# l90lpa/fv3-jedi-linearmodel

Hardware: AMD Instinct MI355X
Metric: column-updates/s per TL+AD dyn step (higher is better)
Workload: dtype f64; 1 GPU; C192L127 hydrostatic TL+AD, six cube faces dealt over 1 GPU(s) (6 per rank), table-driven exchange (221184 columns per GPU), k_split=2 n_split=6 dt=450s nq=4, hord mt/vt/tm/dp/tr=2/2/2/2/2 (sponge: 1/1/1/1 below level 9), kord=17, nord=1; columns_per_gpu=221184

## Files before the change

### fv3_jedi_linearmodel_amd/csrc/tpad.h

```cpp
#pragma once
#include "tpfused.h"

namespace fv3 {
FV3LM_LINK void run_tp_ad(Exec& ex, const TpFusedArgs& a0, const Ctx& c);
}

#if !defined(FV3LM_SPLIT_BUILD) || defined(FV3LM_IMPL_TPAD)
namespace fv3 {

#ifndef FV3LM_TPD_H
#define FV3LM_TPD_H 32
#endif
#if defined(FV3LM_TPD_NOUNROLL) && !defined(FV3LM_HOST_EMUL)
#define TPD_LOOP(e, n) _Pragma("nounroll") for (int e = tid; e < (n); e += NTH)
#define TPD_LOOPU(e, u, n, E) _Pragma("nounroll") for (int e = tid, u = 0; e < (n); e += NTH)
#define TPD_QACC_DIRECT 1
#else
#define TPD_LOOP(e, n) TPF_LOOP(e, n)
#define TPD_LOOPU(e, u, n, E) TPF_LOOPU(e, u, n, E)
#define TPD_QACC_DIRECT 0
#endif
#ifndef FV3LM_TPD_PREFETCH
#define FV3LM_TPD_PREFETCH 1
#endif
#ifndef FV3LM_TPD_EXP
#define FV3LM_TPD_EXP 0
#endif
#ifndef FV3LM_TPD_THREADS
#define FV3LM_TPD_THREADS 1024
#endif
constexpr int TPD_W = 64, TPD_H = FV3LM_TPD_H;
constexpr int TPD_QW = TPD_W + 6, TPD_QH = TPD_H + 6;
constexpr int TPD_AW = TPD_W + 12, TPD_AH = TPD_H + 12;
constexpr int TPD_NQ = TPD_QW * TPD_QH;
constexpr int TPD_NF2 = TPD_QW * (TPD_QH + 1);
constexpr int TPD_NFA = (TPD_AW * TPD_QH > TPD_AH * TPD_QW ? TPD_AW * TPD_QH : TPD_AH * TPD_QW);
constexpr int TPD_NC = TPD_NFA;
constexpr int TPD_NT = 2 * TPD_NQ + TPD_NF2 + 2 * TPD_NFA + TPD_NC;
constexpr int TPD_THREADS = FV3LM_TPD_THREADS;

DEV double tps_al(double fm, double f0, double fp, double cm, double c0, double cp) {
  double s = (c0 > 0. ? (1. - c0) * (1. - c0) : (1. + c0) * (1. + c0)) * f0;
  if (cp > 0.) s -= cp * (1. - cp) * fp;
  if (!(cm > 0.)) s += cm * (1. + cm) * fm;
  return s;
}
template <class D>
DEV double tps_w(bool face, int x, int n1, const D& da, int k) {
  const int e = k - x + 2;
  if (e < 0 || e > 3) return 0.;
  if (!face || (x >= 3 && x <= n1 - 2)) return (e == 0 || e == 3) ? P2 : P1;
  double w[4]; ppm_w(face, x, n1, da, w);
  return w[e];
}
template <class D>
DEV double tps_q(int iord, bool face, int k, int n1, double f0, double fp, double c0, double cp, const double* al, const D& da) {
  double s = 0.;
  if (cp > 0.) s += (iord == 1 ? 1. : cp * (3. - 2. * cp)) * fp;
  if (!(c0 > 0.)) s += (iord == 1 ? 1. : -c0 * (3. + 2. * c0)) * f0;
  if (iord == 1) return s;
  if (!face || (k >= 4 && k <= n1 - 4)) return s + P2 * al[0] + P1 * al[1] + P1 * al[2] + P2 * al[3];
// ... 24 lines not shown
  const double dsc = -Z - (1. - sc) * Y;
  dc = up ? dsc : -dsc;
}

template <int NTH>
DEV void tp_ad_block(const TpFusedArgs& a, const Ctx& c, int tile, int k, int bx, int by, double* lds, int tid, int nth) {
  (void)nth;
  const Geom& g = c.g;
  const int nx = g.nx, ny = g.ny;
  const int is = g.is(), ie = g.ie(), js = g.js(), je = g.je();
  const bool face = g.face != 0;
  const int I0 = is + bx * TPD_W, I1 = (I0 + TPD_W - 1 < ie) ? I0 + TPD_W - 1 : ie;
  const int J0 = js + by * TPD_H, J1 = (J0 + TPD_H - 1 < je) ? J0 + TPD_H - 1 : je;
  const bool firstx = bx == 0, lastx = I1 == ie, firsty = by == 0, lasty = J1 == je;
  const int GI0 = firstx ? I0 - 3 : I0, GI1 = lastx ? I1 + 3 : I1, GJ0 = firsty ? J0 - 3 : J0, GJ1 = lasty ? J1 + 3 : J1;
  const size_t base = (size_t)(tile * a.nk + k - 1) * g.plane;
  auto at = [&](int i, int j) -> size_t { return base + g.idx(i, j); };
  const int iord = hord_of(c.lev[k - 1], a.hsel);
  double* Q = lds;
  double* QG = lds + TPD_NQ;
  double* F2 = lds + 2 * TPD_NQ;
  double* FA = F2 + TPD_NF2;
  double* AL = FA + TPD_NFA;
  double* CT = AL + TPD_NFA;
  auto cxe = [&](int i, int j) { return (j - (J0 - 3)) * TPD_AW + (i - (I0 - 6)); };
  auto cye = [&](int i, int j) { return (j - (J0 - 6)) * TPD_QW + (i - (I0 - 3)); };
  auto load_cx = [&](int e) -> double { const int i = I0 - 6 + e % TPD_AW, j = J0 - 3 + e / TPD_AW; return (i >= is && i <= ie + 1 && i <= I1 + 6 && j <= J1 + 3) ? a.crx.t[at(i, j)] : 0.; };
  auto load_cy = [&](int e) -> double { const int i = I0 - 3 + e % TPD_QW, j = J0 - 6 + e / TPD_QW; return (j >= js && j <= je + 1 && j <= J1 + 6 && i <= I1 + 3) ? a.cry.t[at(i, j)] : 0.; };
#if defined(FV3LM_HOST_EMUL) || defined(FV3LM_TPD_NOUNROLL)
  constexpr bool PRE = false;
#else
  constexpr bool PRE = FV3LM_TPD_PREFETCH != 0;
#endif
#define TPD_PF(arr, u, expr) (PRE ? arr[u] : (expr))
  constexpr int E_AQ = (TPD_AW * TPD_QH + NTH - 1) / NTH, E_QA = (TPD_QW * TPD_AH + NTH - 1) / NTH, E_Q = (TPD_NQ + NTH - 1) / NTH,
                E_V = (TPD_QW * (TPD_H + 1) + NTH - 1) / NTH, E_F = ((TPD_W + 1) * TPD_H + NTH - 1) / NTH,
                E_FB = (TPD_W * (TPD_H + 1) + NTH - 1) / NTH, E_I = (TPD_QW * TPD_H + NTH - 1) / NTH, E_J = (TPD_W * TPD_QH + NTH - 1) / NTH,
                E_G = (TPD_QW * (TPD_QH - 1) + NTH - 1) / NTH, E_GB = ((TPD_QW - 1) * TPD_QH + NTH - 1) / NTH;
#define TPD_SLOTS(E) (PRE ? (E) : 1)
  auto qe = [&](int i, int j) { return (j - (J0 - 3)) * TPD_QW + (i - (I0 - 3)); };
  auto corner_cell = [&](int i, int j) { return face && (i < 1 || i > nx) && (j < 1 || j > ny); };
  constexpr int EQ = (TPD_NQ + NTH - 1) / NTH;
  double qacc[EQ];

  auto cl = [](int m, int n1) { return m < 1 ? 1 : (m > n1 ? n1 : m); };
  (void)cl;
  { constexpr int n = TPD_NQ;
    TPD_LOOP(e, n) { const int i = I0 - 3 + e % TPD_QW, j = J0 - 3 + e / TPD_QW; Q[e] = (i <= I1 + 3 && j <= J1 + 3) ? a.q.t[at(i, j)] : 0.; } }

  {
    auto f2e = [&](int i, int j) { return (j - (J0 - 2)) * TPD_QW + (i - (I0 - 3)); };
    auto fae = [&](int i, int j) { return (j - (J0 - 3)) * TPD_AW + (i - (I0 - 6)); };
    auto ale = [&](int i, int j) { return (j - (J0 - 5)) * TPD_QW + (i - (I0 - 3)); };
    { constexpr int n = TPD_AW * TPD_QH;
      TPD_LOOP(e, n) {
        const int i = I0 - 6 + e % TPD_AW, j = J0 - 3 + e / TPD_AW;
        FA[e] = (i >= is && i <= ie + 1 && j >= js && j <= je && i <= I1 + 6 && j <= J1 + 3) ? 0.5 * a.mx.t[at(i, j)] * a.fx.p[at(i, j)] : 0.;
        CT[e] = load_cx(e);
      } }
    double cv[TPD_SLOTS(E_V)];
    if constexpr (PRE) { constexpr int n = TPD_QW * (TPD_H + 1);
      TPD_LOOPU(e, u, n, E_V) { const int i = I0 - 3 + e % TPD_QW, j = J0 + e / TPD_QW; cv[u] = (i <= I1 + 3 && j <= J1 + 1) ? a.cry.t[at(i, j)] : 0.; } }
    TPF_SYNC();
    double ar2[TPD_SLOTS(E_I)], y02[TPD_SLOTS(E_I)], y12[TPD_SLOTS(E_I)], ry2[TPD_SLOTS(E_I)];
    if constexpr (PRE) { constexpr int n = TPD_QW * TPD_H;
      TPD_LOOPU(e, u, n, E_I) { const int i = I0 - 3 + e % TPD_QW, j = J0 + e / TPD_QW; const bool in = i <= I1 + 3 && j <= J1;
        ar2[u] = in ? MET(area, i, j) : 0.; y02[u] = in ? a.yfx.t[at(i, j)] : 0.; y12[u] = in ? a.yfx.t[at(i, j + 1)] : 0.; ry2[u] = in ? a.ray.t[at(i, j)] : 1.; } }
    { constexpr int n = TPD_QW * (TPD_H + 1);
      TPD_LOOPU(e, u, n, E_V) {
        const int i = I0 - 3 + e % TPD_QW, j = J0 + e / TPD_QW;
        if (i > I1 + 3 || j > J1 + 1) continue;
        auto line = [&](int jj) -> double { int ii = i, j2 = jj; if (face) corner_map(g, 2, ii, j2); return Q[qe(ii, j2)]; };
        const MetY da{c.m.dya, c, tile, i};
        if (FV3LM_TPD_EXP && (a.exp & 1)) { F2[f2e(i, j)] = line(j) * TPD_PF(cv, u, a.cry.t[at(i, j)]); continue; }
        const double cc = TPD_PF(cv, u, a.cry.t[at(i, j)]);
        if (iord == 2 && !(face && (i < 1 || i > nx) && (j <= 3 || j >= ny - 1))) { double v_, d_; tpd_flux2<TPD_QW>(face, j, ny + 1, Q + qe(i, j), cc, da, v_, d_); F2[f2e(i, j)] = v_; }
        else F2[f2e(i, j)] = ppm_flux<double>(iord, face, j, ny + 1, line, da, cc);
      } }
    TPF_SYNC();
    double fx3[TPD_SLOTS(E_F)];
    if constexpr (PRE) { constexpr int w = TPD_W + 1, n = w * TPD_H;
      TPD_LOOPU(e, u, n, E_F) { const int i = I0 + e % w, j = J0 + e / w; fx3[u] = (j <= J1 && (i <= I1 || (lastx && i == I1 + 1))) ? a.fx.p[at(i, j)] : 0.; } }
    { constexpr int n = TPD_QW * TPD_H;
      TPD_LOOPU(e, u, n, E_I) {
        const int i = I0 - 3 + e % TPD_QW, j = J0 + e / TPD_QW;
        if (i > I1 + 3 || j > J1) continue;
        QG[qe(i, j)] = (Q[qe(i, j)] * TPD_PF(ar2, u, MET(area, i, j)) + TPD_PF(y02, u, a.yfx.t[at(i, j)]) * F2[f2e(i, j)] - TPD_PF(y12, u, a.yfx.t[at(i, j + 1)]) * F2[f2e(i, j + 1)]) / TPD_PF(ry2, u, a.ray.t[at(i, j)]);
      } }
    TPF_SYNC();
    double ry4[TPD_SLOTS(E_Q)], ar4[TPD_SLOTS(E_Q)], ro4[TPD_SLOTS(E_Q)];
    if constexpr (PRE) { constexpr int n = TPD_NQ;
      TPD_LOOPU(e, u, n, E_Q) { const int i = I0 - 3 + e % TPD_QW, j = J0 - 3 + e / TPD_QW;
        const bool in = i >= GI0 && i <= GI1 && j >= js && j <= je && j <= J1 + 3, own = in && j >= J0 && j <= J1;
        ry4[u] = in ? a.ray.t[at(i, j)] : 1.; ar4[u] = in ? MET(area, i, j) : 0.; ro4[u] = own ? a.ray.p[at(i, j)] : 0.; } }
    auto FX = [&](int m, int j) { return FA[fae(m, j)]; };
    { constexpr int w = TPD_W + 1, n = w * TPD_H;
      TPD_LOOPU(e, u, n, E_F) {
        const int i = I0 + e % w, j = J0 + e / w;
        if (j > J1 || !(i <= I1 || (lastx && i == I1 + 1))) continue;
        const double fo = FX(i, j), fxad = TPD_PF(fx3, u, a.fx.p[at(i, j)]);
        if (fo == 0. && fxad == 0.) continue;
        if (FV3LM_TPD_EXP && (a.exp & 2)) continue;
        auto line = [&](int ii) -> Dual { return Dual(QG[qe(ii, j)], 0.); };
        const MetX da{c.m.dxa, c, tile, j};
        Dual fl;
        if (iord == 2) tpd_flux2<1>(face, i, nx + 1, QG + qe(i, j), CT[cxe(i, j)], da, fl.v, fl.d);
        else fl = ppm_flux<Dual>(iord, face, i, nx + 1, line, da, Dual(CT[cxe(i, j)], 1.));
        a.crx.p[at(i, j)] += fl.d * fo;
        a.mx.p[at(i, j)] += 0.5 * fl.v * fxad;
      } }
    if (iord == 2 && !(FV3LM_TPD_EXP && (a.exp & 4))) {
      constexpr int n = TPD_AW * TPD_QH;
      TPD_LOOP(e, n) {
        const int x = I0 - 6 + e % TPD_AW, j = J0 - 3 + e / TPD_AW;
        double s = 0.;
        if (x >= I0 - 4 && x <= I1 + 5 && j >= js && j <= je && j <= J1 + 3) s = tps_al(FA[e - 1], FA[e], FA[e + 1], CT[e - 1], CT[e], CT[e + 1]);
        AL[e] = s;
      } }
    TPF_SYNC();
    double yf5[TPD_SLOTS(E_G)], fy5[TPD_SLOTS(E_G)], mm5[TPD_SLOTS(E_G)];
    if constexpr (PRE) { constexpr int n = TPD_QW * (TPD_QH - 1);
      TPD_LOOPU(e, u, n, E_G) { const int i = I0 - 3 + e % TPD_QW, m = J0 - 2 + e / TPD_QW;
        const bool on = i >= GI0 && i <= GI1 && m >= js && m <= je + 1 && m <= J1 + 3, in = on && i >= is && i <= ie;
        yf5[u] = on ? a.yfx.t[at(i, m)] : 0.; fy5[u] = in ? a.fy.p[at(i, m)] : 0.; mm5[u] = in ? a.my.t[at(i, m)] : 0.; } }
    { constexpr int n = TPD_NQ;
      TPD_LOOPU(e, u, n, EQ) {
        const int i = I0 - 3 + e % TPD_QW, j = J0 - 3 + e / TPD_QW;
        double s = 0., acc = 0.;
        if (i >= GI0 && i <= GI1 && j >= js && j <= je && j <= J1 + 3) {
          const bool own = j >= J0 && j <= J1;
          const double ry = TPD_PF(ry4, u, a.ray.t[at(i, j)]), ar = TPD_PF(ar4, u, MET(area, i, j)), rold = TPD_PF(ro4, u, own ? a.ray.p[at(i, j)] : 0.);
          const MetX da{c.m.dxa, c, tile, j};
          const int b0 = fae(i, j);
          if (iord == 333) {
            const double f[4] = {FA[b0 - 1], FA[b0], FA[b0 + 1], FA[b0 + 2]};
            const double cc[4] = {CT[b0 - 1], CT[b0], CT[b0 + 1], CT[b0 + 2]};
            s = tps_q333(face, i, nx + 1, f, cc, da);
          } else {
            const double al[4] = {AL[b0 - 1], AL[b0], AL[b0 + 1], AL[b0 + 2]};
            if (!(FV3LM_TPD_EXP && (a.exp & 8))) s = tps_q(iord, face, i, nx + 1, FA[b0], FA[b0 + 1], CT[b0], CT[b0 + 1], al, da);
          }
          s = s / ry;
          if (own) { a.ray.p[at(i, j)] = rold - QG[e] * s; acc = ar * s; }
        }
        if (TPD_QACC_DIRECT) { if (acc != 0.) a.q.p[at(i, j)] += acc; } else qacc[u] = acc;
        QG[e] = s;
      } }
    TPF_SYNC();
    double cyt[TPD_SLOTS(E_QA)], qo7[TPD_SLOTS(E_Q)];
    if constexpr (PRE) {
      { constexpr int n = TPD_QW * TPD_AH; TPD_LOOPU(e, u, n, E_QA) cyt[u] = load_cy(e); }
      { constexpr int n = TPD_NQ; TPD_LOOPU(e, u, n, E_Q) { const int i = I0 - 3 + e % TPD_QW, j = J0 - 3 + e / TPD_QW;
          qo7[u] = (i < GI0 || i > GI1 || j < GJ0 || j > GJ1 || corner_cell(i, j) || i > I1 + 3 || j > J1 + 3) ? 0. : a.q.p[at(i, j)]; } }
    }
    { constexpr int n = TPD_QW * (TPD_QH - 1);
      TPD_LOOPU(e, u, n, E_G) {
        const int i = I0 - 3 + e % TPD_QW, m = J0 - 2 + e / TPD_QW;
        double s = 0.;
        if (i >= GI0 && i <= GI1 && m >= js && m <= je + 1 && m <= J1 + 3) {
          const bool in = i >= is && i <= ie, own = m >= J0 && (m <= J1 || (lasty && m == J1 + 1));
          const double yf = TPD_PF(yf5, u, a.yfx.t[at(i, m)]), fyad = TPD_PF(fy5, u, in ? a.fy.p[at(i, m)] : 0.), mm = TPD_PF(mm5, u, in ? a.my.t[at(i, m)] : 0.);
          const double dg = (m <= je ? QG[qe(i, m)] : 0.) - (m >= js + 1 ? QG[qe(i, m - 1)] : 0.);
          s = yf * dg + 0.5 * mm * fyad;
          if (own) {
            const double f2v = F2[e];
            a.yfx.p[at(i, m)] += f2v * dg;
            if (in) a.my.p[at(i, m)] += 0.5 * f2v * fyad;
          }
        }
        F2[e] = s;
      } }
    { constexpr int n = TPD_QW * TPD_AH;
      TPD_LOOPU(e, u, n, E_QA) CT[e] = TPD_PF(cyt, u, load_cy(e)); }
    TPF_SYNC();
    auto FY2 = [&](int i, int m) { return (m >= J0 - 2 && m <= J1 + 3) ? F2[f2e(i, m)] : 0.; };
    if (iord == 2 && !(FV3LM_TPD_EXP && (a.exp & 4))) {
      constexpr int n = TPD_QW * TPD_AH;
      TPD_LOOP(e, n) {
        const int i = I0 - 3 + e % TPD_QW, x = J0 - 5 + e / TPD_QW;
        double s = 0.;
        if (i >= GI0 && i <= GI1 && x >= J0 - 4 && x <= J1 + 5) s = tps_al(FY2(i, x - 1), FY2(i, x), FY2(i, x + 1), CT[e], CT[e + TPD_QW], CT[e + 2 * TPD_QW]);
        AL[e] = s;
      } }
    TPF_SYNC();
    { constexpr int n = TPD_NQ;
      TPD_LOOPU(e, u, n, EQ) {
        const int i = I0 - 3 + e % TPD_QW, j = J0 - 3 + e / TPD_QW;
        const double acc = TPD_QACC_DIRECT ? 0. : qacc[u];
        if (i < GI0 || i > GI1 || j < GJ0 || j > GJ1 || corner_cell(i, j)) continue;
        const double qold = TPD_PF(qo7, u, a.q.p[at(i, j)]);
        const MetY da{c.m.dya, c, tile, i};
        const int cb = cye(i, j);
        double s;
        if (iord == 333) {
          const double f[4] = {FY2(i, j - 1), FY2(i, j), FY2(i, j + 1), FY2(i, j + 2)};
          const double cc[4] = {CT[cb - TPD_QW], CT[cb], CT[cb + TPD_QW], CT[cb + 2 * TPD_QW]};
          s = tps_q333(face, j, ny + 1, f, cc, da);
        } else {
          const int b0 = ale(i, j);
          const double al[4] = {AL[b0 - TPD_QW], AL[b0], AL[b0 + TPD_QW], AL[b0 + 2 * TPD_QW]};
          if (!(FV3LM_TPD_EXP && (a.exp & 8))) s = tps_q(iord, face, j, ny + 1, FY2(i, j), FY2(i, j + 1), CT[cb], CT[cb + TPD_QW], al, da);
        }
        a.q.p[at(i, j)] = qold + (acc + s);
      } }
    { constexpr int n = TPD_QW * (TPD_H + 1);
      TPD_LOOP(e, n) {
        const int i = I0 - 3 + e % TPD_QW, m = J0 + e / TPD_QW;
        if (i < GI0 || i > GI1 || !(m <= J1 || (lasty && m == J1 + 1))) continue;
        const double f = F2[f2e(i, m)];
        if (f == 0.) continue;
        if (FV3LM_TPD_EXP && (a.exp & 2)) continue;
        auto line = [&](int jj) -> Dual { int ii = i, j2 = jj; if (face) corner_map(g, 2, ii, j2); return Dual(Q[qe(ii, j2)], 0.); };
        const MetY da{c.m.dya, c, tile, i};
        double v_, d_;
        if (iord == 2 && !(face && (i < 1 || i > nx) && (m <= 3 || m >= ny - 1))) tpd_flux2<TPD_QW>(face, m, ny + 1, Q + qe(i, m), CT[cye(i, m)], da, v_, d_);
        else d_ = ppm_flux<Dual>(iord, face, m, ny + 1, line, da, Dual(CT[cye(i, m)], 1.)).d;
        a.cry.p[at(i, m)] += d_ * f;
      } }
    TPF_SYNC();
  }

  {
    auto f2e = [&](int i, int j) { return (j - (J0 - 3)) * (TPD_QW + 1) + (i - (I0 - 2)); };
    auto fae = [&](int i, int j) { return (j - (J0 - 6)) * TPD_QW + (i - (I0 - 3)); };
    auto ale = [&](int i, int j) { return (j - (J0 - 3)) * TPD_AW + (i - (I0 - 5)); };
    { constexpr int n = TPD_QW * TPD_AH;
      TPD_LOOP(e, n) {
        const int i = I0 - 3 + e % TPD_QW, j = J0 - 6 + e / TPD_QW;
        FA[e] = (j >= js && j <= je + 1 && i >= is && i <= ie && j <= J1 + 6 && i <= I1 + 3) ? 0.5 * a.my.t[at(i, j)] * a.fy.p[at(i, j)] : 0.;
      } }
    double ar2[TPD_SLOTS(E_J)], x02[TPD_SLOTS(E_J)], x12[TPD_SLOTS(E_J)], rx2[TPD_SLOTS(E_J)];
    if constexpr (PRE) { constexpr int n = TPD_W * TPD_QH;
      TPD_LOOPU(e, u, n, E_J) { const int i = I0 + e % TPD_W, j = J0 - 3 + e / TPD_W; const bool in = i <= I1 && j <= J1 + 3;
        ar2[u] = in ? MET(area, i, j) : 0.; x02[u] = in ? a.xfx.t[at(i, j)] : 0.; x12[u] = in ? a.xfx.t[at(i + 1, j)] : 0.; rx2[u] = in ? a.rax.t[at(i, j)] : 1.; } }
    { constexpr int w = TPD_W + 1, n = w * TPD_QH;
      TPD_LOOP(e, n) {
        const int i = I0 + e % w, j = J0 - 3 + e / w;
        if (i > I1 + 1 || j > J1 + 3) continue;
        auto line = [&](int ii) -> double { int i2 = ii, jj = j; if (face) corner_map(g, 1, i2, jj); return Q[qe(i2, jj)]; };
        const MetX da{c.m.dxa, c, tile, j};
        if (FV3LM_TPD_EXP && (a.exp & 1)) { F2[f2e(i, j)] = line(i) * a.crx.t[at(i, j)]; continue; }
        const double cc = a.crx.t[at(i, j)];
        if (iord == 2 && !(face && (j < 1 || j > ny) && (i <= 3 || i >= nx - 1))) { double v_, d_; tpd_flux2<1>(face, i, nx + 1, Q + qe(i, j), cc, da, v_, d_); F2[f2e(i, j)] = v_; }
        else F2[f2e(i, j)] = ppm_flux<double>(iord, face, i, nx + 1, line, da, cc);
      } }
    TPF_SYNC();
    double fy3[TPD_SLOTS(E_FB)];
    if constexpr (PRE) { constexpr int n = TPD_W * (TPD_H + 1);
      TPD_LOOPU(e, u, n, E_FB) { const int i = I0 + e % TPD_W, j = J0 + e / TPD_W; fy3[u] = (i <= I1 && (j <= J1 || (lasty && j == J1 + 1))) ? a.fy.p[at(i, j)] : 0.; } }
    { constexpr int n = TPD_W * TPD_QH;
      TPD_LOOPU(e, u, n, E_J) {
        const int i = I0 + e % TPD_W, j = J0 - 3 + e / TPD_W;
        if (i > I1 || j > J1 + 3) continue;
        QG[qe(i, j)] = (Q[qe(i, j)] * TPD_PF(ar2, u, MET(area, i, j)) + TPD_PF(x02, u, a.xfx.t[at(i, j)]) * F2[f2e(i, j)] - TPD_PF(x12, u, a.xfx.t[at(i + 1, j)]) * F2[f2e(i + 1, j)]) / TPD_PF(rx2, u, a.rax.t[at(i, j)]);
      } }
    TPF_SYNC();
    double rx4[TPD_SLOTS(E_Q)], ar4[TPD_SLOTS(E_Q)], ro4[TPD_SLOTS(E_Q)];
    if constexpr (PRE) { constexpr int n = TPD_NQ;
      TPD_LOOPU(e, u, n, E_Q) { const int i = I0 - 3 + e % TPD_QW, j = J0 - 3 + e / TPD_QW;
        const bool in = j >= GJ0 && j <= GJ1 && i >= is && i <= ie && i <= I1 + 3, own = in && i >= I0 && i <= I1;
        rx4[u] = in ? a.rax.t[at(i, j)] : 1.; ar4[u] = in ? MET(area, i, j) : 0.; ro4[u] = own ? a.rax.p[at(i, j)] : 0.; } }
    auto FY = [&](int i, int m) { return FA[fae(i, m)]; };
    { constexpr int n = TPD_W * (TPD_H + 1);
      TPD_LOOPU(e, u, n, E_FB) {
        const int i = I0 + e % TPD_W, j = J0 + e / TPD_W;
        if (i > I1 || !(j <= J1 || (lasty && j == J1 + 1))) continue;
        const double fo = FY(i, j), fyad = TPD_PF(fy3, u, a.fy.p[at(i, j)]);
        if (fo == 0. && fyad == 0.) continue;
        if (FV3LM_TPD_EXP && (a.exp & 2)) continue;
        auto line = [&](int jj) -> Dual { return Dual(QG[qe(i, jj)], 0.); };
        const MetY da{c.m.dya, c, tile, i};
        Dual fl;
        if (iord == 2) tpd_flux2<TPD_QW>(face, j, ny + 1, QG + qe(i, j), CT[cye(i, j)], da, fl.v, fl.d);
        else fl = ppm_flux<Dual>(iord, face, j, ny + 1, line, da, Dual(CT[cye(i, j)], 1.));
        a.cry.p[at(i, j)] += fl.d * fo;
        a.my.p[at(i, j)] += 0.5 * fl.v * fyad;
      } }
    if (iord == 2 && !(FV3LM_TPD_EXP && (a.exp & 4))) {
      constexpr int n = TPD_QW * TPD_AH;
      TPD_LOOP(e, n) {
        const int i = I0 - 3 + e % TPD_QW, x = J0 - 6 + e / TPD_QW;
        double s = 0.;
        if (x >= J0 - 4 && x <= J1 + 5 && i >= is && i <= ie && i <= I1 + 3) s = tps_al(FA[e - TPD_QW], FA[e], FA[e + TPD_QW], CT[e - TPD_QW], CT[e], CT[e + TPD_QW]);
        AL[e] = s;
      } }
    TPF_SYNC();
    double xf5[TPD_SLOTS(E_GB)], fx5[TPD_SLOTS(E_GB)], mm5[TPD_SLOTS(E_GB)];
    if constexpr (PRE) { constexpr int w = TPD_QW - 1, n = w * TPD_QH;
      TPD_LOOPU(e, u, n, E_GB) { const int m = I0 - 2 + e % w, j = J0 - 3 + e / w;
        const bool on = j >= GJ0 && j <= GJ1 && m >= is && m <= ie + 1 && m <= I1 + 3, in = on && j >= js && j <= je;
        xf5[u] = on ? a.xfx.t[at(m, j)] : 0.; fx5[u] = in ? a.fx.p[at(m, j)] : 0.; mm5[u] = in ? a.mx.t[at(m, j)] : 0.; } }
    { constexpr int n = TPD_NQ;
      TPD_LOOPU(e, u, n, EQ) {
        const int i = I0 - 3 + e % TPD_QW, j = J0 - 3 + e / TPD_QW;
        double s = 0., acc = 0.;
        if (j >= GJ0 && j <= GJ1 && i >= is && i <= ie && i <= I1 + 3) {
          const bool own = i >= I0 && i <= I1;
          const double rx = TPD_PF(rx4, u, a.rax.t[at(i, j)]), ar = TPD_PF(ar4, u, MET(area, i, j)), rold = TPD_PF(ro4, u, own ? a.rax.p[at(i, j)] : 0.);
          const MetY da{c.m.dya, c, tile, i};
          const int b0 = fae(i, j);
          if (iord == 333) {
            const double f[4] = {FA[b0 - TPD_QW], FA[b0], FA[b0 + TPD_QW], FA[b0 + 2 * TPD_QW]};
            const double cc[4] = {CT[b0 - TPD_QW], CT[b0], CT[b0 + TPD_QW], CT[b0 + 2 * TPD_QW]};
            s = tps_q333(face, j, ny + 1, f, cc, da);
          } else {
            const double al[4] = {AL[b0 - TPD_QW], AL[b0], AL[b0 + TPD_QW], AL[b0 + 2 * TPD_QW]};
            if (!(FV3LM_TPD_EXP && (a.exp & 8))) s = tps_q(iord, face, j, ny + 1, FA[b0], FA[b0 + TPD_QW], CT[b0], CT[b0 + TPD_QW], al, da);
          }
          s = s / rx;
          if (own) { a.rax.p[at(i, j)] = rold - QG[e] * s; acc = ar * s; }
        }
        if (TPD_QACC_DIRECT) { if (acc != 0.) a.q.p[at(i, j)] += acc; } else qacc[u] = acc;
        QG[e] = s;
      } }
    TPF_SYNC();
    double cxt[TPD_SLOTS(E_AQ)], qo7[TPD_SLOTS(E_Q)];
    if constexpr (PRE) {
      { constexpr int n = TPD_AW * TPD_QH; TPD_LOOPU(e, u, n, E_AQ) cxt[u] = load_cx(e); }
      { constexpr int n = TPD_NQ; TPD_LOOPU(e, u, n, E_Q) { const int i = I0 - 3 + e % TPD_QW, j = J0 - 3 + e / TPD_QW;
          qo7[u] = (i < GI0 || i > GI1 || j < GJ0 || j > GJ1 || corner_cell(i, j) || i > I1 + 3 || j > J1 + 3) ? 0. : a.q.p[at(i, j)]; } }
    }
    { constexpr int w = TPD_QW - 1, n = w * TPD_QH;
      TPD_LOOPU(e, u, n, E_GB) {
        const int m = I0 - 2 + e % w, j = J0 - 3 + e / w;
        double s = 0.;
        if (j >= GJ0 && j <= GJ1 && m >= is && m <= ie + 1 && m <= I1 + 3) {
          const bool in = j >= js && j <= je, own = m >= I0 && (m <= I1 || (lastx && m == I1 + 1));
          const double xf = TPD_PF(xf5, u, a.xfx.t[at(m, j)]), fxad = TPD_PF(fx5, u, in ? a.fx.p[at(m, j)] : 0.), mm = TPD_PF(mm5, u, in ? a.mx.t[at(m, j)] : 0.);
          const double dg = (m <= ie ? QG[qe(m, j)] : 0.) - (m >= is + 1 ? QG[qe(m - 1, j)] : 0.);
          s = xf * dg + 0.5 * mm * fxad;
          if (own) {
            const double f2v = F2[f2e(m, j)];
            a.xfx.p[at(m, j)] += f2v * dg;
            if (in) a.mx.p[at(m, j)] += 0.5 * f2v * fxad;
          }
        }
        F2[f2e(m, j)] = s;
      } }
    { constexpr int n = TPD_AW * TPD_QH;
      TPD_LOOPU(e, u, n, E_AQ) CT[e] = TPD_PF(cxt, u, load_cx(e)); }
    TPF_SYNC();
    auto FX2 = [&](int m, int j) { return (m >= I0 - 2 && m <= I1 + 3) ? F2[f2e(m, j)] : 0.; };
    if (iord == 2 && !(FV3LM_TPD_EXP && (a.exp & 4))) {
      constexpr int n = TPD_AW * TPD_QH;
      TPD_LOOP(e, n) {
        const int x = I0 - 5 + e % TPD_AW, j = J0 - 3 + e / TPD_AW;
        double s = 0.;
        if (j >= GJ0 && j <= GJ1 && x >= I0 - 4 && x <= I1 + 5) s = tps_al(FX2(x - 1, j), FX2(x, j), FX2(x + 1, j), CT[e], CT[e + 1], CT[e + 2]);
        AL[e] = s;
      } }
    TPF_SYNC();
    { constexpr int n = TPD_NQ;
      TPD_LOOPU(e, u, n, EQ) {
        const int i = I0 - 3 + e % TPD_QW, j = J0 - 3 + e / TPD_QW;
        const double acc = TPD_QACC_DIRECT ? 0. : qacc[u];
        if (i < GI0 || i > GI1 || j < GJ0 || j > GJ1 || corner_cell(i, j)) continue;
        const double qold = TPD_PF(qo7, u, a.q.p[at(i, j)]);
        const MetX da{c.m.dxa, c, tile, j};
        const int cb = cxe(i, j);
        double s;
        if (iord == 333) {
          const double f[4] = {FX2(i - 1, j), FX2(i, j), FX2(i + 1, j), FX2(i + 2, j)};
          const double cc[4] = {CT[cb - 1], CT[cb], CT[cb + 1], CT[cb + 2]};
          s = tps_q333(face, i, nx + 1, f, cc, da);
        } else {
          const int b0 = ale(i, j);
          const double al[4] = {AL[b0 - 1], AL[b0], AL[b0 + 1], AL[b0 + 2]};
          if (!(FV3LM_TPD_EXP && (a.exp & 8))) s = tps_q(iord, face, i, nx + 1, FX2(i, j), FX2(i + 1, j), CT[cb], CT[cb + 1], al, da);
        }
        a.q.p[at(i, j)] = qold + (acc + s);
      } }
    { constexpr int w = TPD_W + 1, n = w * TPD_QH;
      TPD_LOOP(e, n) {
        const int m = I0 + e % w, j = J0 - 3 + e / w;
        if (j < GJ0 || j > GJ1 || j > J1 + 3 || !(m <= I1 || (lastx && m == I1 + 1))) continue;
        const double f = F2[f2e(m, j)];
        if (f == 0.) continue;
        if (FV3LM_TPD_EXP && (a.exp & 2)) continue;
        auto line = [&](int ii) -> Dual { int i2 = ii, jj = j; if (face) corner_map(g, 1, i2, jj); return Dual(Q[qe(i2, jj)], 0.); };
        const MetX da{c.m.dxa, c, tile, j};
        double v_, d_;
        if (iord == 2 && !(face && (j < 1 || j > ny) && (m <= 3 || m >= nx - 1))) tpd_flux2<1>(face, m, nx + 1, Q + qe(m, j), CT[cxe(m, j)], da, v_, d_);
        else d_ = ppm_flux<Dual>(iord, face, m, nx + 1, line, da, Dual(CT[cxe(m, j)], 1.)).d;
        a.crx.p[at(m, j)] += d_ * f;
      } }
  }
#undef TPD_PF
#undef TPD_SLOTS
}

DEV void tp_ad_corner_point(const TpFusedArgs& a, const Ctx& c, int tile, int k, int cn, int n, int dir) {
  const Geom& g = c.g;
  if (!g.face) return;
  const int nx = g.nx, ny = g.ny, ng = g.ng;
  const size_t base = (size_t)(tile * a.nk + k - 1) * g.plane;
  auto at = [&](int i, int j) -> size_t { return base + g.idx(i, j); };
  const int iord = hord_of(c.lev[k - 1], a.hsel);
  const bool west = (cn == 0 || cn == 3), south = (cn < 2);
  if ((west ? g.is() != 1 : g.ie() != nx) || (south ? g.js() != 1 : g.je() != ny)) return;
  int si, sj;
  if (dir == 2) { si = (west ? 1 : nx - ng + 1) + n % ng; sj = (south ? 1 - ng : ny + 1) + n / ng; }
  else { si = (west ? 1 - ng : nx + 1) + n % ng; sj = (south ? 1 : ny - ng + 1) + n / ng; }
  int vi, vj;
  if (!corner_alias(g, dir, si, sj, vi, vj)) return;
  double s = 0.;
  if (dir == 2) {
    const MetY da{c.m.dya, c, tile, vi};
// ... 33 lines not shown
    }
  }
  if (s != 0.) a.q.p[at(si, sj)] += s;
}

#ifndef FV3LM_HOST_EMUL
__global__ void __launch_bounds__(TPD_THREADS) k_tp_ad(TpFusedArgs a, Ctx c) {
  extern __shared__ double tpd_lds[];
  int bx = blockIdx.x, by = blockIdx.y; xcd_block(gridDim.x, gridDim.y, bx, by);
  tp_ad_block<TPD_THREADS>(a, c, blockIdx.z / a.nk, 1 + blockIdx.z % a.nk, bx, by, tpd_lds, threadIdx.x, TPD_THREADS);
}
__global__ void __launch_bounds__(128) k_tp_ad_corner(TpFusedArgs a, Ctx c) {
  const int t = threadIdx.x & 63, dir = threadIdx.x < 64 ? 2 : 1;
  if (t >= 36) return;
  const int tile = blockIdx.x / a.nk, k = 1 + blockIdx.x % a.nk;
  tp_ad_corner_point(a, c, tile, k, t / 9, t % 9, dir);
}
#endif

FV3LM_LINK void run_tp_ad(Exec& ex, const TpFusedArgs& a0, const Ctx& c) {
  TpFusedArgs a = a0;
  for (Fld* f : {&a.q, &a.crx, &a.cry, &a.xfx, &a.yfx, &a.rax, &a.ray, &a.mx, &a.my, &a.fx, &a.fy}) *f = ex.sh(*f);
  const int nbx = (c.g.tx + TPD_W - 1) / TPD_W, nby = (c.g.ty + TPD_H - 1) / TPD_H;
#if FV3LM_TPD_EXP
  if (const char* e = std::getenv("FV3LM_TP2_EXPERIMENT")) a.exp = std::atoi(e);
#endif
  const double cells = double(c.g.tx) * c.g.ty * c.g.ntile * a.nk;
  ex.mark_begin("TpAd", ".ad", 8. * cells * (9. + 2. + 18.));
#ifdef FV3LM_HOST_EMUL
  std::vector<double> lds((size_t)TPD_NT);
  for (int z = 0; z < c.g.ntile * a.nk; ++z)
    for (int by = 0; by < nby; ++by)
      for (int bx = 0; bx < nbx; ++bx) tp_ad_block<1>(a, c, z / a.nk, 1 + z % a.nk, bx, by, lds.data(), 0, 1);
  if (c.g.face)
    for (int z = 0; z < c.g.ntile * a.nk; ++z)
      for (int t = 0; t < 36; ++t) { tp_ad_corner_point(a, c, z / a.nk, 1 + z % a.nk, t / 9, t % 9, 2); tp_ad_corner_point(a, c, z / a.nk, 1 + z % a.nk, t / 9, t % 9, 1); }
#else
  static bool attr = false;
  if (!attr) { if (hipFuncSetAttribute((const void*)k_tp_ad, hipFuncAttributeMaxDynamicSharedMemorySize, TPD_NT * 8) != hipSuccess) set_sticky("hipFuncSetAttribute(k_tp_ad) failed"); attr = true; }
  hipLaunchKernelGGL(k_tp_ad, dim3(nbx, nby, c.g.ntile * a.nk), dim3(TPD_THREADS), TPD_NT * 8, ex.stream, a, c);
#endif
  ex.mark_end();
  ex.launches++;
#ifndef FV3LM_HOST_EMUL
  if (c.g.face) {
    ex.mark_begin("TpAd", ".ad_corner", 0.);
// ... 10 lines not shown
```

Before: 187,000 column-updates/s.

## Keep both Courant halo tiles resident in LDS and prefetch adjoint read-modify-write bases

The single shared CT scratch buffer, which was reloaded from global memory between the y and x passes, is split into separate CX and CY LDS tiles. Both are loaded once at the start and reused in every stage, including the later pass that read crx directly from global. The old values of the adjoint accumulators (crx, cry, mx, my, xfx, yfx) are prefetched into registers before each compute loop, so the `+=` read-modify-writes become plain stores of prefetched value plus increment. This costs more LDS per block and more registers, which may reduce occupancy. It also adds aliasing guards for mx/xfx and my/yfx, and rejects calls where crx aliases mx or cry aliases my.

```diff
diff --git a/fv3_jedi_linearmodel_amd/csrc/tpad.h b/fv3_jedi_linearmodel_amd/csrc/tpad.h
--- a/fv3_jedi_linearmodel_amd/csrc/tpad.h
+++ b/fv3_jedi_linearmodel_amd/csrc/tpad.h
@@ -35,8 +35,8 @@
 constexpr int TPD_NQ = TPD_QW * TPD_QH;
 constexpr int TPD_NF2 = TPD_QW * (TPD_QH + 1);
 constexpr int TPD_NFA = (TPD_AW * TPD_QH > TPD_AH * TPD_QW ? TPD_AW * TPD_QH : TPD_AH * TPD_QW);
-constexpr int TPD_NC = TPD_NFA;
-constexpr int TPD_NT = 2 * TPD_NQ + TPD_NF2 + 2 * TPD_NFA + TPD_NC;
+constexpr int TPD_NCX = TPD_AW * TPD_QH, TPD_NCY = TPD_QW * TPD_AH;
+constexpr int TPD_NT = 2 * TPD_NQ + TPD_NF2 + 2 * TPD_NFA + TPD_NCX + TPD_NCY;
 constexpr int TPD_THREADS = FV3LM_TPD_THREADS;
 
 DEV double tps_al(double fm, double f0, double fp, double cm, double c0, double cp) {
@@ -107,7 +107,8 @@
   double* F2 = lds + 2 * TPD_NQ;
   double* FA = F2 + TPD_NF2;
   double* AL = FA + TPD_NFA;
-  double* CT = AL + TPD_NFA;
+  double* CX = AL + TPD_NFA;
+  double* CY = CX + TPD_NCX;
   auto cxe = [&](int i, int j) { return (j - (J0 - 3)) * TPD_AW + (i - (I0 - 6)); };
   auto cye = [&](int i, int j) { return (j - (J0 - 6)) * TPD_QW + (i - (I0 - 3)); };
   auto load_cx = [&](int e) -> double { const int i = I0 - 6 + e % TPD_AW, j = J0 - 3 + e / TPD_AW; return (i >= is && i <= ie + 1 && i <= I1 + 6 && j <= J1 + 3) ? a.crx.t[at(i, j)] : 0.; };
@@ -118,12 +119,13 @@
   constexpr bool PRE = FV3LM_TPD_PREFETCH != 0;
 #endif
 #define TPD_PF(arr, u, expr) (PRE ? arr[u] : (expr))
-  constexpr int E_AQ = (TPD_AW * TPD_QH + NTH - 1) / NTH, E_QA = (TPD_QW * TPD_AH + NTH - 1) / NTH, E_Q = (TPD_NQ + NTH - 1) / NTH,
-                E_V = (TPD_QW * (TPD_H + 1) + NTH - 1) / NTH, E_F = ((TPD_W + 1) * TPD_H + NTH - 1) / NTH,
+  constexpr int E_Q = (TPD_NQ + NTH - 1) / NTH, E_F = ((TPD_W + 1) * TPD_H + NTH - 1) / NTH,
                 E_FB = (TPD_W * (TPD_H + 1) + NTH - 1) / NTH, E_I = (TPD_QW * TPD_H + NTH - 1) / NTH, E_J = (TPD_W * TPD_QH + NTH - 1) / NTH,
-                E_G = (TPD_QW * (TPD_QH - 1) + NTH - 1) / NTH, E_GB = ((TPD_QW - 1) * TPD_QH + NTH - 1) / NTH;
+                E_G = (TPD_QW * (TPD_QH - 1) + NTH - 1) / NTH, E_GB = ((TPD_QW - 1) * TPD_QH + NTH - 1) / NTH,
+                E_V = (TPD_QW * (TPD_H + 1) + NTH - 1) / NTH, E_X = ((TPD_W + 1) * TPD_QH + NTH - 1) / NTH;
 #define TPD_SLOTS(E) (PRE ? (E) : 1)
   auto qe = [&](int i, int j) { return (j - (J0 - 3)) * TPD_QW + (i - (I0 - 3)); };
+  const bool mx_is_xfx = PRE && a.mx.p == a.xfx.p, my_is_yfx = PRE && a.my.p == a.yfx.p;
   auto corner_cell = [&](int i, int j) { return face && (i < 1 || i > nx) && (j < 1 || j > ny); };
   constexpr int EQ = (TPD_NQ + NTH - 1) / NTH;
   double qacc[EQ];
@@ -141,24 +143,23 @@
       TPD_LOOP(e, n) {
         const int i = I0 - 6 + e % TPD_AW, j = J0 - 3 + e / TPD_AW;
         FA[e] = (i >= is && i <= ie + 1 && j >= js && j <= je && i <= I1 + 6 && j <= J1 + 3) ? 0.5 * a.mx.t[at(i, j)] * a.fx.p[at(i, j)] : 0.;
-        CT[e] = load_cx(e);
-      } }
-    double cv[TPD_SLOTS(E_V)];
-    if constexpr (PRE) { constexpr int n = TPD_QW * (TPD_H + 1);
-      TPD_LOOPU(e, u, n, E_V) { const int i = I0 - 3 + e % TPD_QW, j = J0 + e / TPD_QW; cv[u] = (i <= I1 + 3 && j <= J1 + 1) ? a.cry.t[at(i, j)] : 0.; } }
+        CX[e] = load_cx(e);
+      } }
+    { constexpr int n = TPD_QW * TPD_AH;
+      TPD_LOOP(e, n) CY[e] = load_cy(e); }
     TPF_SYNC();
     double ar2[TPD_SLOTS(E_I)], y02[TPD_SLOTS(E_I)], y12[TPD_SLOTS(E_I)], ry2[TPD_SLOTS(E_I)];
     if constexpr (PRE) { constexpr int n = TPD_QW * TPD_H;
       TPD_LOOPU(e, u, n, E_I) { const int i = I0 - 3 + e % TPD_QW, j = J0 + e / TPD_QW; const bool in = i <= I1 + 3 && j <= J1;
         ar2[u] = in ? MET(area, i, j) : 0.; y02[u] = in ? a.yfx.t[at(i, j)] : 0.; y12[u] = in ? a.yfx.t[at(i, j + 1)] : 0.; ry2[u] = in ? a.ray.t[at(i, j)] : 1.; } }
     { constexpr int n = TPD_QW * (TPD_H + 1);
-      TPD_LOOPU(e, u, n, E_V) {
+      TPD_LOOP(e, n) {
         const int i = I0 - 3 + e % TPD_QW, j = J0 + e / TPD_QW;
         if (i > I1 + 3 || j > J1 + 1) continue;
         auto line = [&](int jj) -> double { int ii = i, j2 = jj; if (face) corner_map(g, 2, ii, j2); return Q[qe(ii, j2)]; };
         const MetY da{c.m.dya, c, tile, i};
-        if (FV3LM_TPD_EXP && (a.exp & 1)) { F2[f2e(i, j)] = line(j) * TPD_PF(cv, u, a.cry.t[at(i, j)]); continue; }
-        const double cc = TPD_PF(cv, u, a.cry.t[at(i, j)]);
+        if (FV3LM_TPD_EXP && (a.exp & 1)) { F2[f2e(i, j)] = line(j) * CY[cye(i, j)]; continue; }
+        const double cc = CY[cye(i, j)];
         if (iord == 2 && !(face && (i < 1 || i > nx) && (j <= 3 || j >= ny - 1))) { double v_, d_; tpd_flux2<TPD_QW>(face, j, ny + 1, Q + qe(i, j), cc, da, v_, d_); F2[f2e(i, j)] = v_; }
         else F2[f2e(i, j)] = ppm_flux<double>(iord, face, j, ny + 1, line, da, cc);
       } }
@@ -179,6 +180,10 @@
         const bool in = i >= GI0 && i <= GI1 && j >= js && j <= je && j <= J1 + 3, own = in && j >= J0 && j <= J1;
         ry4[u] = in ? a.ray.t[at(i, j)] : 1.; ar4[u] = in ? MET(area, i, j) : 0.; ro4[u] = own ? a.ray.p[at(i, j)] : 0.; } }
     auto FX = [&](int m, int j) { return FA[fae(m, j)]; };
+    double co4[TPD_SLOTS(E_F)], mo4[TPD_SLOTS(E_F)];
+    if constexpr (PRE) { constexpr int w = TPD_W + 1, n = w * TPD_H;
+      TPD_LOOPU(e, u, n, E_F) { const int i = I0 + e % w, j = J0 + e / w; const bool own = j <= J1 && (i <= I1 || (lastx && i == I1 + 1));
+        co4[u] = own ? a.crx.p[at(i, j)] : 0.; mo4[u] = own ? a.mx.p[at(i, j)] : 0.; } }
     { constexpr int w = TPD_W + 1, n = w * TPD_H;
       TPD_LOOPU(e, u, n, E_F) {
         const int i = I0 + e % w, j = J0 + e / w;
@@ -189,17 +194,17 @@
         auto line = [&](int ii) -> Dual { return Dual(QG[qe(ii, j)], 0.); };
         const MetX da{c.m.dxa, c, tile, j};
         Dual fl;
-        if (iord == 2) tpd_flux2<1>(face, i, nx + 1, QG + qe(i, j), CT[cxe(i, j)], da, fl.v, fl.d);
-        else fl = ppm_flux<Dual>(iord, face, i, nx + 1, line, da, Dual(CT[cxe(i, j)], 1.));
-        a.crx.p[at(i, j)] += fl.d * fo;
-        a.mx.p[at(i, j)] += 0.5 * fl.v * fxad;
+        if (iord == 2) tpd_flux2<1>(face, i, nx + 1, QG + qe(i, j), CX[cxe(i, j)], da, fl.v, fl.d);
+        else fl = ppm_flux<Dual>(iord, face, i, nx + 1, line, da, Dual(CX[cxe(i, j)], 1.));
+        a.crx.p[at(i, j)] = TPD_PF(co4, u, a.crx.p[at(i, j)]) + fl.d * fo;
+        a.mx.p[at(i, j)] = TPD_PF(mo4, u, a.mx.p[at(i, j)]) + 0.5 * fl.v * fxad;
       } }
     if (iord == 2 && !(FV3LM_TPD_EXP && (a.exp & 4))) {
       constexpr int n = TPD_AW * TPD_QH;
       TPD_LOOP(e, n) {
         const int x = I0 - 6 + e % TPD_AW, j = J0 - 3 + e / TPD_AW;
         double s = 0.;
-        if (x >= I0 - 4 && x <= I1 + 5 && j >= js && j <= je && j <= J1 + 3) s = tps_al(FA[e - 1], FA[e], FA[e + 1], CT[e - 1], CT[e], CT[e + 1]);
+        if (x >= I0 - 4 && x <= I1 + 5 && j >= js && j <= je && j <= J1 + 3) s = tps_al(FA[e - 1], FA[e], FA[e + 1], CX[e - 1], CX[e], CX[e + 1]);
         AL[e] = s;
       } }
     TPF_SYNC();
@@ -219,11 +224,11 @@
           const int b0 = fae(i, j);
           if (iord == 333) {
             const double f[4] = {FA[b0 - 1], FA[b0], FA[b0 + 1], FA[b0 + 2]};
-            const double cc[4] = {CT[b0 - 1], CT[b0], CT[b0 + 1], CT[b0 + 2]};
+            const double cc[4] = {CX[b0 - 1], CX[b0], CX[b0 + 1], CX[b0 + 2]};
             s = tps_q333(face, i, nx + 1, f, cc, da);
           } else {
             const double al[4] = {AL[b0 - 1], AL[b0], AL[b0 + 1], AL[b0 + 2]};
-            if (!(FV3LM_TPD_EXP && (a.exp & 8))) s = tps_q(iord, face, i, nx + 1, FA[b0], FA[b0 + 1], CT[b0], CT[b0 + 1], al, da);
+            if (!(FV3LM_TPD_EXP && (a.exp & 8))) s = tps_q(iord, face, i, nx + 1, FA[b0], FA[b0 + 1], CX[b0], CX[b0 + 1], al, da);
           }
           s = s / ry;
           if (own) { a.ray.p[at(i, j)] = rold - QG[e] * s; acc = ar * s; }
@@ -232,12 +237,16 @@
         QG[e] = s;
       } }
     TPF_SYNC();
-    double cyt[TPD_SLOTS(E_QA)], qo7[TPD_SLOTS(E_Q)];
+    double qo7[TPD_SLOTS(E_Q)];
     if constexpr (PRE) {
-      { constexpr int n = TPD_QW * TPD_AH; TPD_LOOPU(e, u, n, E_QA) cyt[u] = load_cy(e); }
       { constexpr int n = TPD_NQ; TPD_LOOPU(e, u, n, E_Q) { const int i = I0 - 3 + e % TPD_QW, j = J0 - 3 + e / TPD_QW;
           qo7[u] = (i < GI0 || i > GI1 || j < GJ0 || j > GJ1 || corner_cell(i, j) || i > I1 + 3 || j > J1 + 3) ? 0. : a.q.p[at(i, j)]; } }
     }
+    double yo6[TPD_SLOTS(E_G)], mo6[TPD_SLOTS(E_G)];
+    if constexpr (PRE) { constexpr int n = TPD_QW * (TPD_QH - 1);
+      TPD_LOOPU(e, u, n, E_G) { const int i = I0 - 3 + e % TPD_QW, m = J0 - 2 + e / TPD_QW;
+        const bool own = i >= GI0 && i <= GI1 && m >= J0 && (m <= J1 || (lasty && m == J1 + 1)), in = own && i >= is && i <= ie;
+        yo6[u] = own ? a.yfx.p[at(i, m)] : 0.; mo6[u] = (in && !my_is_yfx) ? a.my.p[at(i, m)] : 0.; } }
     { constexpr int n = TPD_QW * (TPD_QH - 1);
       TPD_LOOPU(e, u, n, E_G) {
         const int i = I0 - 3 + e % TPD_QW, m = J0 - 2 + e / TPD_QW;
@@ -249,14 +258,13 @@
           s = yf * dg + 0.5 * mm * fyad;
           if (own) {
             const double f2v = F2[e];
-            a.yfx.p[at(i, m)] += f2v * dg;
-            if (in) a.my.p[at(i, m)] += 0.5 * f2v * fyad;
+            const double y1 = TPD_PF(yo6, u, a.yfx.p[at(i, m)]) + f2v * dg;
+            a.yfx.p[at(i, m)] = y1;
+            if (in) a.my.p[at(i, m)] = (my_is_yfx ? y1 : TPD_PF(mo6, u, a.my.p[at(i, m)])) + 0.5 * f2v * fyad;
           }
         }
         F2[e] = s;
       } }
-    { constexpr int n = TPD_QW * TPD_AH;
-      TPD_LOOPU(e, u, n, E_QA) CT[e] = TPD_PF(cyt, u, load_cy(e)); }
     TPF_SYNC();
     auto FY2 = [&](int i, int m) { return (m >= J0 - 2 && m <= J1 + 3) ? F2[f2e(i, m)] : 0.; };
     if (iord == 2 && !(FV3LM_TPD_EXP && (a.exp & 4))) {
@@ -264,7 +272,7 @@
       TPD_LOOP(e, n) {
         const int i = I0 - 3 + e % TPD_QW, x = J0 - 5 + e / TPD_QW;
         double s = 0.;
-        if (i >= GI0 && i <= GI1 && x >= J0 - 4 && x <= J1 + 5) s = tps_al(FY2(i, x - 1), FY2(i, x), FY2(i, x + 1), CT[e], CT[e + TPD_QW], CT[e + 2 * TPD_QW]);
+        if (i >= GI0 && i <= GI1 && x >= J0 - 4 && x <= J1 + 5) s = tps_al(FY2(i, x - 1), FY2(i, x), FY2(i, x + 1), CY[e], CY[e + TPD_QW], CY[e + 2 * TPD_QW]);
         AL[e] = s;
       } }
     TPF_SYNC();
@@ -279,17 +287,21 @@
         double s;
         if (iord == 333) {
           const double f[4] = {FY2(i, j - 1), FY2(i, j), FY2(i, j + 1), FY2(i, j + 2)};
-          const double cc[4] = {CT[cb - TPD_QW], CT[cb], CT[cb + TPD_QW], CT[cb + 2 * TPD_QW]};
+          const double cc[4] = {CY[cb - TPD_QW], CY[cb], CY[cb + TPD_QW], CY[cb + 2 * TPD_QW]};
           s = tps_q333(face, j, ny + 1, f, cc, da);
         } else {
           const int b0 = ale(i, j);
           const double al[4] = {AL[b0 - TPD_QW], AL[b0], AL[b0 + TPD_QW], AL[b0 + 2 * TPD_QW]};
-          if (!(FV3LM_TPD_EXP && (a.exp & 8))) s = tps_q(iord, face, j, ny + 1, FY2(i, j), FY2(i, j + 1), CT[cb], CT[cb + TPD_QW], al, da);
+          if (!(FV3LM_TPD_EXP && (a.exp & 8))) s = tps_q(iord, face, j, ny + 1, FY2(i, j), FY2(i, j + 1), CY[cb], CY[cb + TPD_QW], al, da);
         }
         a.q.p[at(i, j)] = qold + (acc + s);
       } }
+    double co9[TPD_SLOTS(E_V)];
+    if constexpr (PRE) { constexpr int n = TPD_QW * (TPD_H + 1);
+      TPD_LOOPU(e, u, n, E_V) { const int i = I0 - 3 + e % TPD_QW, m = J0 + e / TPD_QW;
+        co9[u] = (i >= GI0 && i <= GI1 && (m <= J1 || (lasty && m == J1 + 1))) ? a.cry.p[at(i, m)] : 0.; } }
     { constexpr int n = TPD_QW * (TPD_H + 1);
-      TPD_LOOP(e, n) {
+      TPD_LOOPU(e, u, n, E_V) {
         const int i = I0 - 3 + e % TPD_QW, m = J0 + e / TPD_QW;
         if (i < GI0 || i > GI1 || !(m <= J1 || (lasty && m == J1 + 1))) continue;
         const double f = F2[f2e(i, m)];
@@ -298,9 +310,9 @@
         auto line = [&](int jj) -> Dual { int ii = i, j2 = jj; if (face) corner_map(g, 2, ii, j2); return Dual(Q[qe(ii, j2)], 0.); };
         const MetY da{c.m.dya, c, tile, i};
         double v_, d_;
-        if (iord == 2 && !(face && (i < 1 || i > nx) && (m <= 3 || m >= ny - 1))) tpd_flux2<TPD_QW>(face, m, ny + 1, Q + qe(i, m), CT[cye(i, m)], da, v_, d_);
-        else d_ = ppm_flux<Dual>(iord, face, m, ny + 1, line, da, Dual(CT[cye(i, m)], 1.)).d;
-        a.cry.p[at(i, m)] += d_ * f;
+        if (iord == 2 && !(face && (i < 1 || i > nx) && (m <= 3 || m >= ny - 1))) tpd_flux2<TPD_QW>(face, m, ny + 1, Q + qe(i, m), CY[cye(i, m)], da, v_, d_);
+        else d_ = ppm_flux<Dual>(iord, face, m, ny + 1, line, da, Dual(CY[cye(i, m)], 1.)).d;
+        a.cry.p[at(i, m)] = TPD_PF(co9, u, a.cry.p[at(i, m)]) + d_ * f;
       } }
     TPF_SYNC();
   }
@@ -324,8 +336,8 @@
         if (i > I1 + 1 || j > J1 + 3) continue;
         auto line = [&](int ii) -> double { int i2 = ii, jj = j; if (face) corner_map(g, 1, i2, jj); return Q[qe(i2, jj)]; };
         const MetX da{c.m.dxa, c, tile, j};
-        if (FV3LM_TPD_EXP && (a.exp & 1)) { F2[f2e(i, j)] = line(i) * a.crx.t[at(i, j)]; continue; }
-        const double cc = a.crx.t[at(i, j)];
+        if (FV3LM_TPD_EXP && (a.exp & 1)) { F2[f2e(i, j)] = line(i) * CX[cxe(i, j)]; continue; }
+        const double cc = CX[cxe(i, j)];
         if (iord == 2 && !(face && (j < 1 || j > ny) && (i <= 3 || i >= nx - 1))) { double v_, d_; tpd_flux2<1>(face, i, nx + 1, Q + qe(i, j), cc, da, v_, d_); F2[f2e(i, j)] = v_; }
         else F2[f2e(i, j)] = ppm_flux<double>(iord, face, i, nx + 1, line, da, cc);
       } }
@@ -346,6 +358,10 @@
         const bool in = j >= GJ0 && j <= GJ1 && i >= is && i <= ie && i <= I1 + 3, own = in && i >= I0 && i <= I1;
         rx4[u] = in ? a.rax.t[at(i, j)] : 1.; ar4[u] = in ? MET(area, i, j) : 0.; ro4[u] = own ? a.rax.p[at(i, j)] : 0.; } }
     auto FY = [&](int i, int m) { return FA[fae(i, m)]; };
+    double co4[TPD_SLOTS(E_FB)], mo4[TPD_SLOTS(E_FB)];
+    if constexpr (PRE) { constexpr int n = TPD_W * (TPD_H + 1);
+      TPD_LOOPU(e, u, n, E_FB) { const int i = I0 + e % TPD_W, j = J0 + e / TPD_W; const bool own = i <= I1 && (j <= J1 || (lasty && j == J1 + 1));
+        co4[u] = own ? a.cry.p[at(i, j)] : 0.; mo4[u] = own ? a.my.p[at(i, j)] : 0.; } }
     { constexpr int n = TPD_W * (TPD_H + 1);
       TPD_LOOPU(e, u, n, E_FB) {
         const int i = I0 + e % TPD_W, j = J0 + e / TPD_W;
@@ -356,17 +372,17 @@
         auto line = [&](int jj) -> Dual { return Dual(QG[qe(i, jj)], 0.); };
         const MetY da{c.m.dya, c, tile, i};
         Dual fl;
-        if (iord == 2) tpd_flux2<TPD_QW>(face, j, ny + 1, QG + qe(i, j), CT[cye(i, j)], da, fl.v, fl.d);
-        else fl = ppm_flux<Dual>(iord, face, j, ny + 1, line, da, Dual(CT[cye(i, j)], 1.));
-        a.cry.p[at(i, j)] += fl.d * fo;
-        a.my.p[at(i, j)] += 0.5 * fl.v * fyad;
+        if (iord == 2) tpd_flux2<TPD_QW>(face, j, ny + 1, QG + qe(i, j), CY[cye(i, j)], da, fl.v, fl.d);
+        else fl = ppm_flux<Dual>(iord, face, j, ny + 1, line, da, Dual(CY[cye(i, j)], 1.));
+        a.cry.p[at(i, j)] = TPD_PF(co4, u, a.cry.p[at(i, j)]) + fl.d * fo;
+        a.my.p[at(i, j)] = TPD_PF(mo4, u, a.my.p[at(i, j)]) + 0.5 * fl.v * fyad;
       } }
     if (iord == 2 && !(FV3LM_TPD_EXP && (a.exp & 4))) {
       constexpr int n = TPD_QW * TPD_AH;
       TPD_LOOP(e, n) {
         const int i = I0 - 3 + e % TPD_QW, x = J0 - 6 + e / TPD_QW;
         double s = 0.;
-        if (x >= J0 - 4 && x <= J1 + 5 && i >= is && i <= ie && i <= I1 + 3) s = tps_al(FA[e - TPD_QW], FA[e], FA[e + TPD_QW], CT[e - TPD_QW], CT[e], CT[e + TPD_QW]);
+        if (x >= J0 - 4 && x <= J1 + 5 && i >= is && i <= ie && i <= I1 + 3) s = tps_al(FA[e - TPD_QW], FA[e], FA[e + TPD_QW], CY[e - TPD_QW], CY[e], CY[e + TPD_QW]);
         AL[e] = s;
       } }
     TPF_SYNC();
@@ -386,11 +402,11 @@
           const int b0 = fae(i, j);
           if (iord == 333) {
             const double f[4] = {FA[b0 - TPD_QW], FA[b0], FA[b0 + TPD_QW], FA[b0 + 2 * TPD_QW]};
-            const double cc[4] = {CT[b0 - TPD_QW], CT[b0], CT[b0 + TPD_QW], CT[b0 + 2 * TPD_QW]};
+            const double cc[4] = {CY[b0 - TPD_QW], CY[b0], CY[b0 + TPD_QW], CY[b0 + 2 * TPD_QW]};
             s = tps_q333(face, j, ny + 1, f, cc, da);
           } else {
             const double al[4] = {AL[b0 - TPD_QW], AL[b0], AL[b0 + TPD_QW], AL[b0 + 2 * TPD_QW]};
-            if (!(FV3LM_TPD_EXP && (a.exp & 8))) s = tps_q(iord, face, j, ny + 1, FA[b0], FA[b0 + TPD_QW], CT[b0], CT[b0 + TPD_QW], al, da);
+            if (!(FV3LM_TPD_EXP && (a.exp & 8))) s = tps_q(iord, face, j, ny + 1, FA[b0], FA[b0 + TPD_QW], CY[b0], CY[b0 + TPD_QW], al, da);
           }
           s = s / rx;
           if (own) { a.rax.p[at(i, j)] = rold - QG[e] * s; acc = ar * s; }
@@ -399,12 +415,16 @@
         QG[e] = s;
       } }
     TPF_SYNC();
-    double cxt[TPD_SLOTS(E_AQ)], qo7[TPD_SLOTS(E_Q)];
+    double qo7[TPD_SLOTS(E_Q)];
     if constexpr (PRE) {
-      { constexpr int n = TPD_AW * TPD_QH; TPD_LOOPU(e, u, n, E_AQ) cxt[u] = load_cx(e); }
       { constexpr int n = TPD_NQ; TPD_LOOPU(e, u, n, E_Q) { const int i = I0 - 3 + e % TPD_QW, j = J0 - 3 + e / TPD_QW;
           qo7[u] = (i < GI0 || i > GI1 || j < GJ0 || j > GJ1 || corner_cell(i, j) || i > I1 + 3 || j > J1 + 3) ? 0. : a.q.p[at(i, j)]; } }
     }
+    double xo6[TPD_SLOTS(E_GB)], mo6[TPD_SLOTS(E_GB)];
+    if constexpr (PRE) { constexpr int w = TPD_QW - 1, n = w * TPD_QH;
+      TPD_LOOPU(e, u, n, E_GB) { const int m = I0 - 2 + e % w, j = J0 - 3 + e / w;
+        const bool own = j >= GJ0 && j <= GJ1 && m >= I0 && (m <= I1 || (lastx && m == I1 + 1)), in = own && j >= js && j <= je;
+        xo6[u] = own ? a.xfx.p[at(m, j)] : 0.; mo6[u] = (in && !mx_is_xfx) ? a.mx.p[at(m, j)] : 0.; } }
     { constexpr int w = TPD_QW - 1, n = w * TPD_QH;
       TPD_LOOPU(e, u, n, E_GB) {
         const int m = I0 - 2 + e % w, j = J0 - 3 + e / w;
@@ -416,14 +436,13 @@
           s = xf * dg + 0.5 * mm * fxad;
           if (own) {
             const double f2v = F2[f2e(m, j)];
-            a.xfx.p[at(m, j)] += f2v * dg;
-            if (in) a.mx.p[at(m, j)] += 0.5 * f2v * fxad;
+            const double x1 = TPD_PF(xo6, u, a.xfx.p[at(m, j)]) + f2v * dg;
+            a.xfx.p[at(m, j)] = x1;
+            if (in) a.mx.p[at(m, j)] = (mx_is_xfx ? x1 : TPD_PF(mo6, u, a.mx.p[at(m, j)])) + 0.5 * f2v * fxad;
           }
         }
         F2[f2e(m, j)] = s;
       } }
-    { constexpr int n = TPD_AW * TPD_QH;
-      TPD_LOOPU(e, u, n, E_AQ) CT[e] = TPD_PF(cxt, u, load_cx(e)); }
     TPF_SYNC();
     auto FX2 = [&](int m, int j) { return (m >= I0 - 2 && m <= I1 + 3) ? F2[f2e(m, j)] : 0.; };
     if (iord == 2 && !(FV3LM_TPD_EXP && (a.exp & 4))) {
@@ -431,7 +450,7 @@
       TPD_LOOP(e, n) {
         const int x = I0 - 5 + e % TPD_AW, j = J0 - 3 + e / TPD_AW;
         double s = 0.;
-        if (j >= GJ0 && j <= GJ1 && x >= I0 - 4 && x <= I1 + 5) s = tps_al(FX2(x - 1, j), FX2(x, j), FX2(x + 1, j), CT[e], CT[e + 1], CT[e + 2]);
+        if (j >= GJ0 && j <= GJ1 && x >= I0 - 4 && x <= I1 + 5) s = tps_al(FX2(x - 1, j), FX2(x, j), FX2(x + 1, j), CX[e], CX[e + 1], CX[e + 2]);
         AL[e] = s;
       } }
     TPF_SYNC();
@@ -446,17 +465,21 @@
         double s;
         if (iord == 333) {
           const double f[4] = {FX2(i - 1, j), FX2(i, j), FX2(i + 1, j), FX2(i + 2, j)};
-          const double cc[4] = {CT[cb - 1], CT[cb], CT[cb + 1], CT[cb + 2]};
+          const double cc[4] = {CX[cb - 1], CX[cb], CX[cb + 1], CX[cb + 2]};
           s = tps_q333(face, i, nx + 1, f, cc, da);
         } else {
           const int b0 = ale(i, j);
           const double al[4] = {AL[b0 - 1], AL[b0], AL[b0 + 1], AL[b0 + 2]};
-          if (!(FV3LM_TPD_EXP && (a.exp & 8))) s = tps_q(iord, face, i, nx + 1, FX2(i, j), FX2(i + 1, j), CT[cb], CT[cb + 1], al, da);
+          if (!(FV3LM_TPD_EXP && (a.exp & 8))) s = tps_q(iord, face, i, nx + 1, FX2(i, j), FX2(i + 1, j), CX[cb], CX[cb + 1], al, da);
         }
         a.q.p[at(i, j)] = qold + (acc + s);
       } }
+    double co9[TPD_SLOTS(E_X)];
+    if constexpr (PRE) { constexpr int w = TPD_W + 1, n = w * TPD_QH;
+      TPD_LOOPU(e, u, n, E_X) { const int m = I0 + e % w, j = J0 - 3 + e / w;
+        co9[u] = (j >= GJ0 && j <= GJ1 && (m <= I1 || (lastx && m == I1 + 1))) ? a.crx.p[at(m, j)] : 0.; } }
     { constexpr int w = TPD_W + 1, n = w * TPD_QH;
-      TPD_LOOP(e, n) {
+      TPD_LOOPU(e, u, n, E_X) {
         const int m = I0 + e % w, j = J0 - 3 + e / w;
         if (j < GJ0 || j > GJ1 || j > J1 + 3 || !(m <= I1 || (lastx && m == I1 + 1))) continue;
         const double f = F2[f2e(m, j)];
@@ -465,9 +488,9 @@
         auto line = [&](int ii) -> Dual { int i2 = ii, jj = j; if (face) corner_map(g, 1, i2, jj); return Dual(Q[qe(i2, jj)], 0.); };
         const MetX da{c.m.dxa, c, tile, j};
         double v_, d_;
-        if (iord == 2 && !(face && (j < 1 || j > ny) && (m <= 3 || m >= nx - 1))) tpd_flux2<1>(face, m, nx + 1, Q + qe(m, j), CT[cxe(m, j)], da, v_, d_);
-        else d_ = ppm_flux<Dual>(iord, face, m, nx + 1, line, da, Dual(CT[cxe(m, j)], 1.)).d;
-        a.crx.p[at(m, j)] += d_ * f;
+        if (iord == 2 && !(face && (j < 1 || j > ny) && (m <= 3 || m >= nx - 1))) tpd_flux2<1>(face, m, nx + 1, Q + qe(m, j), CX[cxe(m, j)], da, v_, d_);
+        else d_ = ppm_flux<Dual>(iord, face, m, nx + 1, line, da, Dual(CX[cxe(m, j)], 1.)).d;
+        a.crx.p[at(m, j)] = TPD_PF(co9, u, a.crx.p[at(m, j)]) + d_ * f;
       } }
   }
 #undef TPD_PF
@@ -547,6 +570,7 @@
   TpFusedArgs a = a0;
   for (Fld* f : {&a.q, &a.crx, &a.cry, &a.xfx, &a.yfx, &a.rax, &a.ray, &a.mx, &a.my, &a.fx, &a.fy}) *f = ex.sh(*f);
   const int nbx = (c.g.tx + TPD_W - 1) / TPD_W, nby = (c.g.ty + TPD_H - 1) / TPD_H;
+  if (a.crx.p == a.mx.p || a.cry.p == a.my.p) { set_sticky("run_tp_ad: crx_ad / mx_ad or cry_ad / my_ad are one array"); return; }
 #if FV3LM_TPD_EXP
   if (const char* e = std::getenv("FV3LM_TP2_EXPERIMENT")) a.exp = std::atoi(e);
 #endif
```

Result: no change. 186,000 column-updates/s (-0.5%).
